# OFA-Sys/ONE-PEACE

Hardware: NVIDIA H100
Metric: encoder_samples_per_sec (higher is better)
Workload: dtype bf16

## Files before the change

one_peace_b200/csrc/gemm_wgmma.cu:

```cuda
#include "common.cuh"
#include "gemm.h"

#include <mutex>

namespace opb {

constexpr int kBlockM = 128;
constexpr int kBlockN = 256;
constexpr int kBlockK = 64;
constexpr int kStages = 4;
constexpr int kABytes = kBlockM * kBlockK * 2;
constexpr int kBBytes = kBlockN * kBlockK * 2;
constexpr int kStageBytes = kABytes + kBBytes;
constexpr int kThreads = 384;
constexpr int kBandM = 8;
constexpr int kResidBatch = 16;

struct EpiOperands {
  float2 row[kBlockM];
  float colsum[kBlockN], bias[kBlockN], gamma[kBlockN], colscale[kBlockN];
};
constexpr int kStagerThreads = 96;
constexpr int kSmemBytes = kStages * kStageBytes + 1024 + 2 * sizeof(EpiOperands) + 1024;

struct GemmGeom {
  int M, N, K;
  int kb_inner;
  int num_k_blocks;
  int groups;
  int a_group_c0;
  int b_group_rows;
  int a_mn;
  int b_mn;
  int kb_per_piece;
  int m_pad;
  float* split_ws;
};

OPB_DEVICE void fence_acc(float (&d)[128]) {
#pragma unroll
  for (int i = 0; i < 128; ++i) asm volatile("" : "+f"(d[i])::"memory");
}

template <int TA, int TB>
OPB_DEVICE void wgmma_m64n256k16(float (&d)[128], uint64_t desc_a, uint64_t desc_b, uint32_t scale_d) {
  asm volatile(
      "{\n\t"
      ".reg .pred p;\n\t"
      "setp.ne.b32 p, %130, 0;\n\t"
      "wgmma.mma_async.sync.aligned.m64n256k16.f32.bf16.bf16 "
      "{"
      "%0, %1, %2, %3, %4, %5, %6, %7, %8, %9, %10, %11, %12, %13, %14, %15, "
      "%16, %17, %18, %19, %20, %21, %22, %23, %24, %25, %26, %27, %28, %29, %30, %31, "
      "%32, %33, %34, %35, %36, %37, %38, %39, %40, %41, %42, %43, %44, %45, %46, %47, "
      "%48, %49, %50, %51, %52, %53, %54, %55, %56, %57, %58, %59, %60, %61, %62, %63, "
      "%64, %65, %66, %67, %68, %69, %70, %71, %72, %73, %74, %75, %76, %77, %78, %79, "
      "%80, %81, %82, %83, %84, %85, %86, %87, %88, %89, %90, %91, %92, %93, %94, %95, "
      "%96, %97, %98, %99, %100, %101, %102, %103, %104, %105, %106, %107, %108, %109, %110, %111, "
      "%112, %113, %114, %115, %116, %117, %118, %119, %120, %121, %122, %123, %124, %125, %126, %127"
      "}, %128, %129, p, 1, 1, %131, %132;\n\t"
      "}\n"
      : "+f"(d[0]), "+f"(d[1]), "+f"(d[2]), "+f"(d[3]), "+f"(d[4]), "+f"(d[5]), "+f"(d[6]), "+f"(d[7]),
        "+f"(d[8]), "+f"(d[9]), "+f"(d[10]), "+f"(d[11]), "+f"(d[12]), "+f"(d[13]), "+f"(d[14]), "+f"(d[15]),
        "+f"(d[16]), "+f"(d[17]), "+f"(d[18]), "+f"(d[19]), "+f"(d[20]), "+f"(d[21]), "+f"(d[22]), "+f"(d[23]),
        "+f"(d[24]), "+f"(d[25]), "+f"(d[26]), "+f"(d[27]), "+f"(d[28]), "+f"(d[29]), "+f"(d[30]), "+f"(d[31]),
        "+f"(d[32]), "+f"(d[33]), "+f"(d[34]), "+f"(d[35]), "+f"(d[36]), "+f"(d[37]), "+f"(d[38]), "+f"(d[39]),
        "+f"(d[40]), "+f"(d[41]), "+f"(d[42]), "+f"(d[43]), "+f"(d[44]), "+f"(d[45]), "+f"(d[46]), "+f"(d[47]),
        "+f"(d[48]), "+f"(d[49]), "+f"(d[50]), "+f"(d[51]), "+f"(d[52]), "+f"(d[53]), "+f"(d[54]), "+f"(d[55]),
        "+f"(d[56]), "+f"(d[57]), "+f"(d[58]), "+f"(d[59]), "+f"(d[60]), "+f"(d[61]), "+f"(d[62]), "+f"(d[63]),
        "+f"(d[64]), "+f"(d[65]), "+f"(d[66]), "+f"(d[67]), "+f"(d[68]), "+f"(d[69]), "+f"(d[70]), "+f"(d[71]),
        "+f"(d[72]), "+f"(d[73]), "+f"(d[74]), "+f"(d[75]), "+f"(d[76]), "+f"(d[77]), "+f"(d[78]), "+f"(d[79]),
        "+f"(d[80]), "+f"(d[81]), "+f"(d[82]), "+f"(d[83]), "+f"(d[84]), "+f"(d[85]), "+f"(d[86]), "+f"(d[87]),
        "+f"(d[88]), "+f"(d[89]), "+f"(d[90]), "+f"(d[91]), "+f"(d[92]), "+f"(d[93]), "+f"(d[94]), "+f"(d[95]),
        "+f"(d[96]), "+f"(d[97]), "+f"(d[98]), "+f"(d[99]), "+f"(d[100]), "+f"(d[101]), "+f"(d[102]), "+f"(d[103]),
        "+f"(d[104]), "+f"(d[105]), "+f"(d[106]), "+f"(d[107]), "+f"(d[108]), "+f"(d[109]), "+f"(d[110]), "+f"(d[111]),
        "+f"(d[112]), "+f"(d[113]), "+f"(d[114]), "+f"(d[115]), "+f"(d[116]), "+f"(d[117]), "+f"(d[118]), "+f"(d[119]),
        "+f"(d[120]), "+f"(d[121]), "+f"(d[122]), "+f"(d[123]), "+f"(d[124]), "+f"(d[125]), "+f"(d[126]), "+f"(d[127])
      : "l"(desc_a), "l"(desc_b), "r"(scale_d), "n"(TA), "n"(TB));
}

template <bool kFusedVar = false>
OPB_DEVICE void load_ln_stats(const GemmEpilogue& ep, int row, int M, float& mu, float& rs) {
  mu = 0.f; rs = 1.f;
  const int rc = row < M ? row : M - 1;
  if (ep.ln_partial != nullptr) {
    float s1 = 0.f, s2 = 0.f;
#pragma unroll 8
    for (int p = 0; p < ep.ln_parts; ++p) {
      const float2 v = *reinterpret_cast<const float2*>(ep.ln_partial + (static_cast<long>(p) * M + rc) * 2);
// ... 20 lines not shown
                         uint32_t it0) {
  constexpr uint32_t step_a = TA ? 2048 : 32, step_b = TB ? 2048 : 32;
  const bool signal = (threadIdx.x & 31) == 0;
  for (int kb = 0; kb < num_k_blocks; ++kb) {
    const uint32_t it = it0 + kb;
    const uint32_t s = it % kStages;
    mbar_wait_quiet(&full[s], (it / kStages) & 1);
    const uint32_t sa = smem_u32(smem + s * kStageBytes) + cw * 8192;
    const uint32_t sb = smem_u32(smem + s * kStageBytes + kABytes);
    fence_acc(d);
    wgmma_fence();
#pragma unroll
    for (int k = 0; k < kBlockK / 16; ++k)
      wgmma_m64n256k16<TA, TB>(d, wgmma_desc_sw128(sa + k * step_a, 8192), wgmma_desc_sw128(sb + k * step_b, 8192),
                               (kb > 0 || k > 0) ? 1u : 0u);
    wgmma_commit();
    fence_acc(d);
    if (kb > 0) {
      wgmma_wait<1>();
      fence_acc(d);
      __syncwarp();
      if (signal) mbar_arrive(&empty[(it - 1) % kStages]);
    }
  }
  wgmma_wait<0>();
  fence_acc(d);
  __syncwarp();
  if (signal) mbar_arrive(&empty[(it0 + num_k_blocks - 1) % kStages]);
}

constexpr bool epi_staged(int epi) { return epi != EPI_LSE_PARTIAL && epi != EPI_SOFTMAX_GRAD; }

template <int EPI>
OPB_DEVICE void stage_epi_operands(EpiOperands* st, const GemmEpilogue& ep, const GemmGeom& geo, int m_blk, int n_blk, int grp,
                                   int t) {
  if (ep.ln_partial != nullptr || ep.ln_mu != nullptr) {
    for (int r = t; r < kBlockM; r += kStagerThreads) {
      float mu, rs;
      load_ln_stats<EPI == EPI_GEGLU_BF16 || EPI == EPI_RESID_F32>(ep, m_blk * kBlockM + r, geo.M, mu, rs);
      st->row[r] = make_float2(mu, rs);
    }
  }
  for (int c = t; c < kBlockN; c += kStagerThreads) {
    const int tc = n_blk * kBlockN + c;
    const bool ok = tc < geo.N;
    const int col = grp * geo.N + tc;
    st->colsum[c] = ok && ep.ln_colsum != nullptr ? ep.ln_colsum[col] : 0.f;
    st->bias[c] = ok && ep.bias != nullptr ? ep.bias[col] : 0.f;
    st->gamma[c] = ok && ep.gamma != nullptr ? ep.gamma[col] : 0.f;
    st->colscale[c] = ok && ep.colscale != nullptr ? ep.colscale[col] : 0.f;
  }
}

template <int EPI>
OPB_DEVICE void epilogue(const float (&d)[128], const GemmEpilogue& ep, const GemmGeom& geo, const EpiOperands* st, int m_blk,
                         int n_blk, int grp, int cw) {
  const int M = geo.M, N = geo.N;
  const int t = threadIdx.x & 127;
  const int lane = t & 31;
  const int quad = lane & 3;
  const int rloc = cw * 64 + (t >> 5) * 16 + (lane >> 2);
  const int rbase = m_blk * kBlockM + rloc;
  const int col0 = n_blk * kBlockN;
  const int gcol0 = grp * N;
#pragma unroll
  for (int h = 0; h < 2; ++h) {
    const int row = rbase + 8 * h;
    bool row_ok = row < M;
    if (ep.out_group > 0 && ep.out_group_valid > 0 && (row % ep.out_group) >= ep.out_group_valid) row_ok = false;
    long out_row = row;
    if (ep.out_group > 0) out_row = static_cast<long>(row / ep.out_group) * ep.out_group_stride + (row % ep.out_group) + ep.out_row_offset;
    long res_row = out_row;
    if (ep.resid_period > 0) res_row = (row % ep.resid_period) + ep.resid_row_offset;

    if constexpr (EPI == EPI_LSE_PARTIAL) {
      const float scale = *ep.scale_ptr;
      const int tgt = row + ep.target_offset;
      const int nv = ep.n_valid > 0 ? ep.n_valid : N;
      float m = -INFINITY;
#pragma unroll
      for (int j = 0; j < 32; ++j) {
        const int col = col0 + 8 * j + 2 * quad;
        if (col < nv) m = fmaxf(m, scale * d[4 * j + 2 * h]);
        if (col + 1 < nv) m = fmaxf(m, scale * d[4 * j + 2 * h + 1]);
      }
      float ssum = 0.f, zsum = 0.f, best = -INFINITY, ztgt = 0.f;
      int best_idx = 0, has_tgt = 0;
#pragma unroll
      for (int j = 0; j < 32; ++j) {
#pragma unroll
        for (int e = 0; e < 2; ++e) {
          const int col = col0 + 8 * j + 2 * quad + e;
          if (col < nv) {
            const float z = scale * d[4 * j + 2 * h + e];
            ssum += __expf(z - m);
            zsum += z;
            if (z > best) { best = z; best_idx = col; }
            if (col == tgt) { ztgt = z; has_tgt = 1; }
          }
        }
      }
#pragma unroll
      for (int o = 1; o <= 2; o <<= 1) {
        const float m2 = __shfl_xor_sync(0xffffffffu, m, o), s2 = __shfl_xor_sync(0xffffffffu, ssum, o);
        const float zs2 = __shfl_xor_sync(0xffffffffu, zsum, o), b2 = __shfl_xor_sync(0xffffffffu, best, o);
        const int i2 = __shfl_xor_sync(0xffffffffu, best_idx, o), h2 = __shfl_xor_sync(0xffffffffu, has_tgt, o);
        const float zt2 = __shfl_xor_sync(0xffffffffu, ztgt, o);
        const float mn = fmaxf(m, m2);
        ssum = (m > -INFINITY ? ssum * __expf(m - mn) : 0.f) + (m2 > -INFINITY ? s2 * __expf(m2 - mn) : 0.f);
        m = mn;
        zsum += zs2;
        if (b2 > best || (b2 == best && i2 < best_idx)) { best = b2; best_idx = i2; }
        if (h2) { ztgt = zt2; has_tgt = 1; }
      }
      if (row_ok && quad == 0) {
        float* w = ep.ws + (static_cast<long>(n_blk) * M + row) * 8;
        *reinterpret_cast<float4*>(w) = make_float4(m, ssum, zsum, best);
        *reinterpret_cast<float4*>(w + 4) = make_float4(__int_as_float(best_idx), ztgt, has_tgt ? 1.f : 0.f, 0.f);
      }
    } else if constexpr (EPI == EPI_SOFTMAX_GRAD) {
      const float scale = *ep.scale_ptr;
      const float gscale = scale * ep.coef;
      const int tgt = row + ep.target_offset;
      const float lse = row_ok ? ep.row_lse[row] : 0.f;
      const float hit = 1.f - ep.eps - ep.eps_i;
      const int nv = ep.n_valid > 0 ? ep.n_valid : N;
      float gz = 0.f;
#pragma unroll
      for (int j = 0; j < 32; ++j) {
        const int col = col0 + 8 * j + 2 * quad;
        if (!row_ok || col >= N) continue;
        float gq[2];
#pragma unroll
        for (int e = 0; e < 2; ++e) {
          const float z = scale * d[4 * j + 2 * h + e];
          float g = __expf(z - lse) - ep.eps_i;
          if (col + e == tgt) g -= hit;
          if (col + e >= nv) g = 0.f;
          gz += g * z;
          gq[e] = g * gscale;
        }
        *reinterpret_cast<uint32_t*>(reinterpret_cast<__nv_bfloat16*>(ep.out) + out_row * ep.ldo + col) = pack_bf16x2(gq[0], gq[1]);
      }
      gz = quad_sum(gz);
      if (row_ok && quad == 0) ep.ws[static_cast<long>(n_blk) * M + row] = gz;
    } else {
      const float2 mr = (ep.ln_partial != nullptr || ep.ln_mu != nullptr) ? st->row[rloc + 8 * h] : make_float2(0.f, 1.f);
      const float mu = mr.x, rs = mr.y;
      const bool has_ln = ep.ln_colsum != nullptr;
      float st_sum = 0.f, st_sq = 0.f;
      if constexpr (EPI == EPI_GEGLU_BF16) {
        __nv_bfloat16* out = reinterpret_cast<__nv_bfloat16*>(ep.out) + out_row * ep.ldo + n_blk * (kBlockN / 2);
#pragma unroll
        for (int j = 0; j < 16; ++j) {
          const int tc = 8 * j + 2 * quad;
          float g0 = d[4 * j + 2 * h], g1 = d[4 * j + 2 * h + 1];
          float l0 = d[4 * (j + 16) + 2 * h], l1 = d[4 * (j + 16) + 2 * h + 1];
          if (has_ln) {
            const float2 cg = ldf2(st->colsum + tc), cl = ldf2(st->colsum + tc + kBlockN / 2);
            g0 = rs * (g0 - mu * cg.x); g1 = rs * (g1 - mu * cg.y);
            l0 = rs * (l0 - mu * cl.x); l1 = rs * (l1 - mu * cl.y);
          }
          if (ep.bias != nullptr) {
            const float2 bg = ldf2(st->bias + tc), bl = ldf2(st->bias + tc + kBlockN / 2);
            g0 += bg.x; g1 += bg.y; l0 += bl.x; l1 += bl.y;
          }
          const float u0 = gelu_erf(g0) * l0, u1 = gelu_erf(g1) * l1;
          st_sum += u0 + u1;
          st_sq += u0 * u0 + u1 * u1;
          if (row_ok) *reinterpret_cast<uint32_t*>(out + tc) = pack_bf16x2(u0, u1);
        }
        st_sum = quad_sum(st_sum);
        st_sq = quad_sum(st_sq);
        if (row_ok && quad == 0 && ep.stats_out != nullptr) {
          *reinterpret_cast<float2*>(ep.stats_out + (static_cast<long>(n_blk * 2) * M + row) * 2) = make_float2(st_sum, st_sq);
          *reinterpret_cast<float2*>(ep.stats_out + (static_cast<long>(n_blk * 2 + 1) * M + row) * 2) = make_float2(0.f, 0.f);
        }
      } else {
#pragma unroll
        for (int jb = 0; jb < 32; jb += kResidBatch) {
          float2 res[kResidBatch];
          if constexpr (EPI == EPI_RESID_F32) {
            if (ep.resid != nullptr && row_ok) {
              const float* rp = ep.resid + res_row * ep.ldr + gcol0;
#pragma unroll
              for (int jj = 0; jj < kResidBatch; ++jj) {
                const int tc = col0 + 8 * (jb + jj) + 2 * quad;
                if (tc < N) res[jj] = ldf2(rp + tc);
              }
            }
          }
#pragma unroll
          for (int jj = 0; jj < kResidBatch; ++jj) {
            const int j = jb + jj;
            const int lc = 8 * j + 2 * quad;
            const int tc = col0 + lc;
            if (tc >= N) continue;
            const int col = gcol0 + tc;
            float x0 = d[4 * j + 2 * h], x1 = d[4 * j + 2 * h + 1];
            if (has_ln) {
              const float2 c = ldf2(st->colsum + lc);
              x0 = rs * (x0 - mu * c.x); x1 = rs * (x1 - mu * c.y);
            }
            if (ep.bias != nullptr) {
              const float2 b = ldf2(st->bias + lc);
              x0 += b.x; x1 += b.y;
            }
            if constexpr (EPI == EPI_STORE_BF16 || EPI == EPI_GELU_BF16) {
              if (ep.colscale != nullptr) {
                const float2 s = ldf2(st->colscale + lc);
                x0 *= s.x; x1 *= s.y;
              }
              if constexpr (EPI == EPI_GELU_BF16) { x0 = gelu_erf(x0); x1 = gelu_erf(x1); }
              if (row_ok) *reinterpret_cast<uint32_t*>(reinterpret_cast<__nv_bfloat16*>(ep.out) + out_row * ep.ldo + col) = pack_bf16x2(x0, x1);
            } else {
              if constexpr (EPI == EPI_RESID_F32) {
                if (ep.gamma != nullptr) {
                  const float2 g = ldf2(st->gamma + lc);
                  x0 *= g.x; x1 *= g.y;
                }
                if (ep.resid != nullptr && row_ok) {
                  x0 += res[jj].x; x1 += res[jj].y;
                }
                st_sum += x0 + x1;
                st_sq += x0 * x0 + x1 * x1;
                if (row_ok && ep.out_bf16 != nullptr)
                  *reinterpret_cast<uint32_t*>(reinterpret_cast<__nv_bfloat16*>(ep.out_bf16) + out_row * ep.ldo_bf16 + col) = pack_bf16x2(x0, x1);
              }
              if (row_ok) *reinterpret_cast<float2*>(reinterpret_cast<float*>(ep.out) + out_row * ep.ldo + col) = make_float2(x0, x1);
            }
          }
        }
        if constexpr (EPI == EPI_RESID_F32) {
          st_sum = quad_sum(st_sum);
          st_sq = quad_sum(st_sq);
          if (row_ok && quad == 0 && ep.stats_out != nullptr)
            *reinterpret_cast<float2*>(ep.stats_out + (static_cast<long>(n_blk) * M + row) * 2) = make_float2(st_sum, st_sq);
        }
      }
    }
  }
}

struct TileCoord {
  int piece, grp, m_blk, n_blk;
};
OPB_DEVICE TileCoord tile_coord(int unit, int num_m_tiles, int num_n_tiles, int groups) {
  const int per_group = num_m_tiles * num_n_tiles;
  TileCoord c;
  c.piece = unit / (per_group * groups);
  const int tile = unit - c.piece * per_group * groups;
  c.grp = tile / per_group;
  const int tin = tile - c.grp * per_group;
  const int band = tin / (kBandM * num_n_tiles);
  const int m0 = band * kBandM;
  const int band_rows = min(kBandM, num_m_tiles - m0);
  const int r = tin - m0 * num_n_tiles;
  c.m_blk = m0 + r % band_rows;
  c.n_blk = r / band_rows;
  return c;
}

template <int EPI>
__global__ void __launch_bounds__(kThreads, 1)
gemm_bf16_kernel(const __grid_constant__ CUtensorMap tm_a, const __grid_constant__ CUtensorMap tm_b, const GemmEpilogue ep,
                 const GemmGeom geo) {
  extern __shared__ __align__(1024) uint8_t smem_raw[];
  uint8_t* smem = smem_raw;
  if ((smem_u32(smem) & 1023u) != 0) __trap();
  uint64_t* full = reinterpret_cast<uint64_t*>(smem + kStages * kStageBytes);
  uint64_t* empty = full + kStages;
  uint64_t* epi_full = empty + kStages;
  uint64_t* epi_empty = epi_full + 2;
  EpiOperands* epi_ops = reinterpret_cast<EpiOperands*>(smem + kStages * kStageBytes + 1024);

  const int wg = threadIdx.x >> 7;
  const int num_m_tiles = (geo.M + kBlockM - 1) / kBlockM;
  const int num_n_tiles = (geo.N + kBlockN - 1) / kBlockN;
  const int pieces = geo.kb_per_piece > 0 ? (geo.num_k_blocks + geo.kb_per_piece - 1) / geo.kb_per_piece : 1;
  const int units = num_m_tiles * num_n_tiles * geo.groups * pieces;
  const bool staged = epi_staged(EPI) && geo.kb_per_piece == 0;

  if (threadIdx.x == 0) {
    tma_prefetch_desc(&tm_a);
    tma_prefetch_desc(&tm_b);
    for (int i = 0; i < kStages; ++i) {
      mbar_init(&full[i], 1);
      mbar_init(&empty[i], 8);
    }
    for (int i = 0; i < 2; ++i) {
      mbar_init(&epi_full[i], kStagerThreads);
      mbar_init(&epi_empty[i], 8);
    }
    fence_barrier_init();
  }
  __syncthreads();

  if (wg == 0) {
    asm volatile("setmaxnreg.dec.sync.aligned.u32 40;");
    if (threadIdx.x == 0) {
      uint32_t it = 0;
      for (int unit = blockIdx.x; unit < units; unit += gridDim.x) {
        const TileCoord tc = tile_coord(unit, num_m_tiles, num_n_tiles, geo.groups);
        const int kb0 = geo.kb_per_piece > 0 ? tc.piece * geo.kb_per_piece : 0;
        const int kb1 = geo.kb_per_piece > 0 ? min(geo.num_k_blocks, kb0 + geo.kb_per_piece) : geo.num_k_blocks;
        const int a_row = tc.m_blk * kBlockM;
        const int b_row = tc.grp * geo.b_group_rows + tc.n_blk * kBlockN;
        const int a_c0 = tc.grp * geo.a_group_c0;
        int kin = kb0 % geo.kb_inner, tap = kb0 / geo.kb_inner;
        for (int kb = kb0; kb < kb1; ++kb, ++it) {
          const uint32_t s = it % kStages;
          mbar_wait_quiet(&empty[s], ((it / kStages) & 1) ^ 1);
          uint8_t* sa = smem + s * kStageBytes;
          uint8_t* sb = sa + kABytes;
          mbar_arrive_expect_tx(&full[s], kStageBytes);
          if (geo.a_mn) {
#pragma unroll
            for (int i = 0; i < kBlockM / 64; ++i) tma_load_2d(&tm_a, &full[s], sa + i * 8192, a_row + 64 * i, kb * kBlockK);
          } else {
            tma_load_3d(&tm_a, &full[s], sa, a_c0 + kin * kBlockK, tap, a_row);
          }
          if (geo.b_mn) {
#pragma unroll
            for (int i = 0; i < kBlockN / 64; ++i) tma_load_2d(&tm_b, &full[s], sb + i * 8192, b_row + 64 * i, kb * kBlockK);
          } else {
            tma_load_2d(&tm_b, &full[s], sb, kb * kBlockK, b_row);
          }
          if (++kin == geo.kb_inner) { kin = 0; ++tap; }
        }
      }
    } else if (threadIdx.x >= 32 && staged) {
      uint32_t j = 0;
      for (int unit = blockIdx.x; unit < units; unit += gridDim.x, ++j) {
        const TileCoord tc = tile_coord(unit, num_m_tiles, num_n_tiles, geo.groups);
        mbar_wait_quiet(&epi_empty[j & 1], ((j >> 1) & 1) ^ 1);
        stage_epi_operands<EPI>(&epi_ops[j & 1], ep, geo, tc.m_blk, tc.n_blk, tc.grp, threadIdx.x - 32);
        mbar_arrive(&epi_full[j & 1]);
      }
    }
  } else {
    asm volatile("setmaxnreg.inc.sync.aligned.u32 232;");
    const int cw = wg - 1;
    float d[128];
#pragma unroll
    for (int i = 0; i < 128; ++i) d[i] = 0.f;
    uint32_t it = 0, j = 0;
    for (int unit = blockIdx.x; unit < units; unit += gridDim.x, ++j) {
      const TileCoord tc = tile_coord(unit, num_m_tiles, num_n_tiles, geo.groups);
      const int kb0 = geo.kb_per_piece > 0 ? tc.piece * geo.kb_per_piece : 0;
      const int kb1 = geo.kb_per_piece > 0 ? min(geo.num_k_blocks, kb0 + geo.kb_per_piece) : geo.num_k_blocks;
      if (geo.a_mn) {
        if (geo.b_mn) mainloop<1, 1>(d, smem, full, empty, kb1 - kb0, cw, it);
        else mainloop<1, 0>(d, smem, full, empty, kb1 - kb0, cw, it);
      } else {
        if (geo.b_mn) mainloop<0, 1>(d, smem, full, empty, kb1 - kb0, cw, it);
        else mainloop<0, 0>(d, smem, full, empty, kb1 - kb0, cw, it);
      }
      it += kb1 - kb0;
      if (geo.kb_per_piece > 0) {
        const int t = threadIdx.x & 127, lane = t & 31;
        const int r0 = tc.m_blk * kBlockM + cw * 64 + (t >> 5) * 16 + (lane >> 2);
        float* w = geo.split_ws + static_cast<long>(tc.piece) * geo.m_pad * geo.N;
#pragma unroll
        for (int h = 0; h < 2; ++h) {
#pragma unroll
          for (int c = 0; c < 32; ++c) {
            const int col = tc.n_blk * kBlockN + 8 * c + 2 * (lane & 3);
            if (col < geo.N)
              *reinterpret_cast<float2*>(w + static_cast<long>(r0 + 8 * h) * geo.N + col) = make_float2(d[4 * c + 2 * h], d[4 * c + 2 * h + 1]);
          }
        }
      } else if (staged) {
        mbar_wait_quiet(&epi_full[j & 1], (j >> 1) & 1);
        epilogue<EPI>(d, ep, geo, &epi_ops[j & 1], tc.m_blk, tc.n_blk, tc.grp, cw);
        __syncwarp();
        if ((threadIdx.x & 31) == 0) mbar_arrive(&epi_empty[j & 1]);
      } else {
        epilogue<EPI>(d, ep, geo, nullptr, tc.m_blk, tc.n_blk, tc.grp, cw);
      }
    }
  }
}

__global__ void __launch_bounds__(256)
gemm_split_epilogue_kernel(const GemmEpilogue ep, const GemmGeom geo, int pieces, int epi) {
  __shared__ float red[2][8];
  const int M = geo.M, N = geo.N;
  const int row = blockIdx.x;
  float mu, rs;
  if (ep.ln_partial != nullptr) {
    float s1 = 0.f, s2 = 0.f;
    for (int p = threadIdx.x; p < ep.ln_parts; p += blockDim.x) {
      const float2 v = *reinterpret_cast<const float2*>(ep.ln_partial + (static_cast<long>(p) * M + row) * 2);
      s1 += v.x; s2 += v.y;
    }
    s1 = warp_sum(s1); s2 = warp_sum(s2);
    if ((threadIdx.x & 31) == 0) { red[0][threadIdx.x >> 5] = s1; red[1][threadIdx.x >> 5] = s2; }
    __syncthreads();
    s1 = s2 = 0.f;
    for (int i = 0; i < 8; ++i) { s1 += red[0][i]; s2 += red[1][i]; }
    mu = s1 / ep.ln_dim;
    rs = rsqrtf(fmaxf(s2 / ep.ln_dim - mu * mu, 0.f) + ep.ln_eps);
  } else {
    load_ln_stats(ep, row, M, mu, rs);
  }
  const int t = blockIdx.y;
  const int col = t * kBlockN + threadIdx.x;
  const long slab = static_cast<long>(geo.m_pad) * N;
  float x = 0.f;
  if (col < N) {
    const float* w = geo.split_ws + static_cast<long>(row) * N + col;
    for (int p = 0; p < pieces; ++p) x += w[p * slab];
    if (ep.ln_colsum) x = rs * (x - mu * ep.ln_colsum[col]);
    if (ep.bias) x += ep.bias[col];
    if (epi == EPI_STORE_BF16) {
      if (ep.colscale) x *= ep.colscale[col];
      reinterpret_cast<__nv_bfloat16*>(ep.out)[static_cast<long>(row) * ep.ldo + col] = __float2bfloat16(x);
    } else {
      if (ep.gamma) x *= ep.gamma[col];
      if (ep.resid) x += ep.resid[static_cast<long>(row) * ep.ldr + col];
      reinterpret_cast<float*>(ep.out)[static_cast<long>(row) * ep.ldo + col] = x;
      if (ep.out_bf16) reinterpret_cast<__nv_bfloat16*>(ep.out_bf16)[static_cast<long>(row) * ep.ldo_bf16 + col] = __float2bfloat16(x);
    }
  }
  if (ep.stats_out != nullptr) {
    const float s1 = warp_sum(x), s2 = warp_sum(x * x);
    __syncthreads();
    if ((threadIdx.x & 31) == 0) { red[0][threadIdx.x >> 5] = s1; red[1][threadIdx.x >> 5] = s2; }
    __syncthreads();
    if (threadIdx.x == 0) {
      float a = 0.f, b = 0.f;
// ... 38 lines not shown

int make_tmap_bf16_3d(CUtensorMap* out, const void* ptr, uint64_t k_inner, uint64_t taps, uint64_t tap_stride,
                      uint64_t rows, uint64_t row_stride, uint32_t box_rows) {
  PFN_encodeTiled enc = get_encode_fn();
  if (enc == nullptr) return OPB_ERR_CUDA;
  if ((reinterpret_cast<uintptr_t>(ptr) & 15) != 0 || (tap_stride * 2) % 16 != 0 || (row_stride * 2) % 16 != 0)
    return OPB_ERR_INVALID;
  cuuint64_t gdim[3] = {k_inner, taps, rows};
  cuuint64_t gstride[2] = {tap_stride * 2, row_stride * 2};
  cuuint32_t box[3] = {static_cast<cuuint32_t>(kBlockK), 1, box_rows};
  cuuint32_t estr[3] = {1, 1, 1};
  CUresult r = enc(out, CU_TENSOR_MAP_DATA_TYPE_BFLOAT16, 3, const_cast<void*>(ptr), gdim, gstride, box, estr,
                   CU_TENSOR_MAP_INTERLEAVE_NONE, CU_TENSOR_MAP_SWIZZLE_128B, CU_TENSOR_MAP_L2_PROMOTION_L2_256B,
                   CU_TENSOR_MAP_FLOAT_OOB_FILL_NONE);
  return r == CUDA_SUCCESS ? OPB_OK : OPB_ERR_CUDA;
}

int make_tmap_bf16_batched(CUtensorMap* out, const void* ptr, uint64_t cols, uint64_t rows, uint64_t ld, uint64_t batches,
                           uint64_t batch_stride, uint32_t box_rows) {
  PFN_encodeTiled enc = get_encode_fn();
  if (enc == nullptr) return OPB_ERR_CUDA;
  if ((reinterpret_cast<uintptr_t>(ptr) & 15) != 0 || (ld * 2) % 16 != 0 || (batch_stride * 2) % 16 != 0)
    return OPB_ERR_INVALID;
  cuuint64_t gdim[3] = {cols, rows, batches};
  cuuint64_t gstride[2] = {ld * 2, batch_stride * 2};
  cuuint32_t box[3] = {static_cast<cuuint32_t>(kBlockK), box_rows, 1};
  cuuint32_t estr[3] = {1, 1, 1};
  CUresult r = enc(out, CU_TENSOR_MAP_DATA_TYPE_BFLOAT16, 3, const_cast<void*>(ptr), gdim, gstride, box, estr,
                   CU_TENSOR_MAP_INTERLEAVE_NONE, CU_TENSOR_MAP_SWIZZLE_128B, CU_TENSOR_MAP_L2_PROMOTION_L2_256B,
                   CU_TENSOR_MAP_FLOAT_OOB_FILL_NONE);
  return r == CUDA_SUCCESS ? OPB_OK : OPB_ERR_CUDA;
}

template <int EPI>
static int launch_gemm(const CUtensorMap& ta, const CUtensorMap& tb, const GemmEpilogue& ep, const GemmGeom& geo,
                       cudaStream_t stream) {
  auto kern = gemm_bf16_kernel<EPI>;
  static int resident = 0;
  if (resident == 0) {
    if (cudaFuncSetAttribute(kern, cudaFuncAttributeMaxDynamicSharedMemorySize, kSmemBytes) != cudaSuccess)
      return OPB_ERR_CUDA;
    int per_sm = 0;
    if (cudaOccupancyMaxActiveBlocksPerMultiprocessor(&per_sm, kern, kThreads, kSmemBytes) != cudaSuccess || per_sm < 1)
      return OPB_ERR_CUDA;
    resident = per_sm * sm_count();
  }
  const int pieces = geo.kb_per_piece > 0 ? (geo.num_k_blocks + geo.kb_per_piece - 1) / geo.kb_per_piece : 1;
  const long units = static_cast<long>((geo.M + kBlockM - 1) / kBlockM) * ((geo.N + kBlockN - 1) / kBlockN) * geo.groups * pieces;
  const unsigned grid = static_cast<unsigned>(units < resident ? units : resident);
  kern<<<grid, kThreads, kSmemBytes, stream>>>(ta, tb, ep, geo);
  return cudaGetLastError() == cudaSuccess ? OPB_OK : OPB_ERR_CUDA;
}

static int dispatch_gemm(int epi, const CUtensorMap& ta, const CUtensorMap& tb, const GemmEpilogue& ep, const GemmGeom& geo,
                         cudaStream_t stream) {
  switch (epi) {
    case EPI_STORE_BF16: return launch_gemm<EPI_STORE_BF16>(ta, tb, ep, geo, stream);
    case EPI_GELU_BF16: return launch_gemm<EPI_GELU_BF16>(ta, tb, ep, geo, stream);
    case EPI_GEGLU_BF16: return launch_gemm<EPI_GEGLU_BF16>(ta, tb, ep, geo, stream);
    case EPI_RESID_F32: return launch_gemm<EPI_RESID_F32>(ta, tb, ep, geo, stream);
    case EPI_STORE_F32: return launch_gemm<EPI_STORE_F32>(ta, tb, ep, geo, stream);
    case EPI_LSE_PARTIAL: return launch_gemm<EPI_LSE_PARTIAL>(ta, tb, ep, geo, stream);
    case EPI_SOFTMAX_GRAD: return launch_gemm<EPI_SOFTMAX_GRAD>(ta, tb, ep, geo, stream);
    default: return OPB_ERR_INVALID;
  }
}

struct ByteSpan {
  const char* begin;
  const char* end;
};
static ByteSpan row_span(const void* p, long lo, long hi, long ld, long cols, int esz) {
  const char* c = static_cast<const char*>(p);
  return {c + lo * ld * esz, c + (hi * ld + cols) * esz};
}
static bool spans_meet(const ByteSpan& a, const ByteSpan& b) { return a.begin < b.end && b.begin < a.end; }

static bool resid_aliasing_ok(const GemmEpilogue& ep, int M, long cols) {
  if (ep.resid == nullptr) return true;
  auto out_row = [&](long m) {
    return ep.out_group > 0 ? (m / ep.out_group) * ep.out_group_stride + m % ep.out_group + ep.out_row_offset : m;
  };
  const long g = ep.out_group > 0 ? ep.out_group : M, last = M - 1, q = last / g;
  const long corners[5] = {0, (g < M ? g : M) - 1, q * g, last, q > 0 ? q * g - 1 : 0};
  long lo = out_row(0), hi = lo;
  for (long m : corners) {
    lo = out_row(m) < lo ? out_row(m) : lo;
    hi = out_row(m) > hi ? out_row(m) : hi;
  }
  long rlo = lo, rhi = hi;
  if (ep.resid_period > 0) {
    rlo = ep.resid_row_offset;
    rhi = rlo + (ep.resid_period < M ? ep.resid_period : M) - 1;
  }
  const ByteSpan res = row_span(ep.resid, rlo, rhi, ep.ldr, cols, 4);
  if (ep.out_bf16 != nullptr && spans_meet(res, row_span(ep.out_bf16, lo, hi, ep.ldo_bf16, cols, 2))) return false;
  if (!spans_meet(res, row_span(ep.out, lo, hi, ep.ldo, cols, 4))) return true;
  return ep.resid == ep.out && ep.ldr == ep.ldo && ep.resid_period == 0;
}

static GemmGeom plain_geom(int M, int N, int K) {
  GemmGeom geo;
  geo.M = M; geo.N = N; geo.K = K;
  geo.num_k_blocks = (K + kBlockK - 1) / kBlockK;
  geo.kb_inner = geo.num_k_blocks;
  geo.groups = 1;
  geo.a_group_c0 = 0;
  geo.b_group_rows = 0;
  geo.a_mn = geo.b_mn = 0;
  geo.kb_per_piece = 0;
  geo.m_pad = 0;
  geo.split_ws = nullptr;
  return geo;
}

int gemm_bf16(const void* A, int lda, const void* B, int ldb, int M, int N, int K, int epi, const GemmEpilogue& ep,
              int cta_group, cudaStream_t stream) {
  if (M <= 0 || N <= 0 || K <= 0) return OPB_ERR_INVALID;
  if (K % 8 != 0 || N % 8 != 0 || lda % 8 != 0 || ldb % 8 != 0) return OPB_ERR_INVALID;
  if (epi == EPI_GEGLU_BF16 && N % kBlockN != 0) return OPB_ERR_INVALID;
  if (cta_group < 0 || cta_group > 2) return OPB_ERR_INVALID;
  if (epi == EPI_RESID_F32 && !resid_aliasing_ok(ep, M, N)) return OPB_ERR_INVALID;
  GemmGeom geo = plain_geom(M, N, K);
  const int m_tiles = (M + kBlockM - 1) / kBlockM, n_tiles = (N + kBlockN - 1) / kBlockN;
  const bool split_ok = (epi == EPI_RESID_F32 || (epi == EPI_STORE_BF16 && ep.stats_out == nullptr)) && ep.workspace != nullptr &&
                        ep.out_group == 0 && ep.resid_period == 0 && M <= 2 * kBlockM && geo.num_k_blocks >= 8;
  int pieces = 1;
  if (split_ok) {
    const long slab_bytes = static_cast<long>(m_tiles) * kBlockM * N * 4;
    pieces = sm_count() / (m_tiles * n_tiles);
    if (pieces > geo.num_k_blocks / 2) pieces = geo.num_k_blocks / 2;
    if (pieces > ep.workspace_bytes / slab_bytes) pieces = static_cast<int>(ep.workspace_bytes / slab_bytes);
    if (pieces >= 2) {
      geo.kb_per_piece = (geo.num_k_blocks + pieces - 1) / pieces;
      pieces = (geo.num_k_blocks + geo.kb_per_piece - 1) / geo.kb_per_piece;
      geo.m_pad = m_tiles * kBlockM;
      geo.split_ws = reinterpret_cast<float*>(ep.workspace);
    }
  }
  CUtensorMap ta, tb;
  int rc = make_tmap_bf16_3d(&ta, A, K, 1, lda, M, lda, kBlockM);
  if (rc != OPB_OK) return rc;
  rc = make_tmap_bf16_2d(&tb, B, N, K, ldb, kBlockN);
  if (rc != OPB_OK) return rc;
  rc = dispatch_gemm(epi, ta, tb, ep, geo, stream);
  if (rc != OPB_OK || geo.kb_per_piece == 0) return rc;
  gemm_split_epilogue_kernel<<<dim3(M, n_tiles), 256, 0, stream>>>(ep, geo, pieces, epi);
  return cudaGetLastError() == cudaSuccess ? OPB_OK : OPB_ERR_CUDA;
}

int gemm_bf16_t(const void* A, int lda, int a_mn, const void* B, int ldb, int b_mn, int M, int N, int K, int epi,
                const GemmEpilogue& ep, int cta_group, cudaStream_t stream) {
  if (M <= 0 || N <= 0 || K <= 0 || lda % 8 != 0 || ldb % 8 != 0 || N % 8 != 0) return OPB_ERR_INVALID;
  if (epi != EPI_STORE_BF16 && epi != EPI_STORE_F32) return OPB_ERR_INVALID;
  if ((!a_mn && K % 8 != 0) || (!b_mn && K % 8 != 0) || (a_mn && M % 8 != 0)) return OPB_ERR_INVALID;
  if (cta_group < 0 || cta_group > 2) return OPB_ERR_INVALID;
  GemmGeom geo = plain_geom(M, N, K);
  geo.a_mn = a_mn ? 1 : 0;
  geo.b_mn = b_mn ? 1 : 0;
  CUtensorMap ta, tb;
  int rc = a_mn ? make_tmap_bf16_2d(&ta, A, K, M, lda, 64) : make_tmap_bf16_3d(&ta, A, K, 1, lda, M, lda, kBlockM);
  if (rc != OPB_OK) return rc;
  rc = b_mn ? make_tmap_bf16_2d(&tb, B, K, N, ldb, 64) : make_tmap_bf16_2d(&tb, B, N, K, ldb, kBlockN);
  if (rc != OPB_OK) return rc;
  return dispatch_gemm(epi, ta, tb, ep, geo, stream);
// ... 25 lines not shown
```

Measured before the change: 760.6.

## Stage GEMM epilogue outputs through swizzled per-warp smem for coalesced 16B stores

```diff
diff --git a/one_peace_b200/csrc/gemm_wgmma.cu b/one_peace_b200/csrc/gemm_wgmma.cu
--- a/one_peace_b200/csrc/gemm_wgmma.cu
+++ b/one_peace_b200/csrc/gemm_wgmma.cu
@@ -1,6 +1,7 @@
 #include "common.cuh"
 #include "gemm.h"
 
+#include <algorithm>
 #include <mutex>
 
 namespace opb {
@@ -14,14 +15,15 @@
 constexpr int kStageBytes = kABytes + kBBytes;
 constexpr int kThreads = 384;
 constexpr int kBandM = 8;
-constexpr int kResidBatch = 16;
 
 struct EpiOperands {
   float2 row[kBlockM];
   float colsum[kBlockN], bias[kBlockN], gamma[kBlockN], colscale[kBlockN];
 };
 constexpr int kStagerThreads = 96;
-constexpr int kSmemBytes = kStages * kStageBytes + 1024 + 2 * sizeof(EpiOperands) + 1024;
+constexpr int kWarpStageBytes = 16 * 128;
+constexpr int kSmemBytes = kStages * kStageBytes + 1024 + 2 * sizeof(EpiOperands) + 8 * kWarpStageBytes + 1024;
+static_assert(kSmemBytes <= 232448, "exceeds the sm_90 opt-in shared memory per block");
 
 struct GemmGeom {
   int M, N, K;
@@ -35,6 +37,7 @@
   int kb_per_piece;
   int m_pad;
   float* split_ws;
+  int vec;
 };
 
 OPB_DEVICE void fence_acc(float (&d)[128]) {
@@ -161,28 +164,79 @@
   }
 }
 
+OPB_DEVICE int stage_off(int r, int byte) {
+  const int swz = ((r & 3) << 1) | ((r >> 2) & 1);
+  return r * 128 + ((((byte >> 4) ^ swz) << 4) | (byte & 15));
+}
+OPB_DEVICE void stage_bf16x2(uint8_t* buf, int r, int jj, int quad, float a, float b) {
+  *reinterpret_cast<uint32_t*>(buf + stage_off(r, jj * 16 + quad * 4)) = pack_bf16x2(a, b);
+}
+OPB_DEVICE void stage_f32x2(uint8_t* buf, int r, int jj, int quad, float a, float b) {
+  *reinterpret_cast<float2*>(buf + stage_off(r, jj * 32 + quad * 8)) = make_float2(a, b);
+}
+
+OPB_DEVICE void st_global_vec(char* p, const uint4& v, int bytes, int vec) {
+  if (vec == 16) {
+    *reinterpret_cast<uint4*>(p) = v;
+    return;
+  }
+  const uint32_t w[4] = {v.x, v.y, v.z, v.w};
+#pragma unroll
+  for (int i = 0; i < 4; ++i) {
+    if (4 * i >= bytes) break;
+    if (vec == 8) {
+      if ((i & 1) == 0) *reinterpret_cast<uint2*>(p + 4 * i) = make_uint2(w[i], w[i + 1]);
+    } else {
+      *reinterpret_cast<uint32_t*>(p + 4 * i) = w[i];
+    }
+  }
+}
+
+OPB_DEVICE void unstage(const uint8_t* buf, int drow, char* out, long ld, int valid, int vec,
+                        char* out_bf16 = nullptr, long ld_bf16 = 0) {
+  const int lane = threadIdx.x & 31;
+  const int b = (lane & 7) * 16;
+  __syncwarp();
+#pragma unroll
+  for (int i = 0; i < 4; ++i) {
+    const int r = 4 * i + (lane >> 3);
+    const uint4 v = *reinterpret_cast<const uint4*>(buf + stage_off(r, b));
+    const int orow = __shfl_sync(0xffffffffu, drow, r);
+    if (orow < 0 || b >= valid) continue;
+    st_global_vec(out + static_cast<long>(orow) * ld + b, v, 16, vec);
+    if (out_bf16 != nullptr) {
+      const uint4 h = make_uint4(pack_bf16x2(__uint_as_float(v.x), __uint_as_float(v.y)),
+                                 pack_bf16x2(__uint_as_float(v.z), __uint_as_float(v.w)), 0u, 0u);
+      st_global_vec(out_bf16 + static_cast<long>(orow) * ld_bf16 + b / 2, h, 8, vec / 2);
+    }
+  }
+  __syncwarp();
+}
+
+OPB_DEVICE int out_row_of(const GemmEpilogue& ep, int row, int M) {
+  if (row >= M) return -1;
+  if (ep.out_group <= 0) return row;
+  if (ep.out_group_valid > 0 && row % ep.out_group >= ep.out_group_valid) return -1;
+  return (row / ep.out_group) * ep.out_group_stride + row % ep.out_group + ep.out_row_offset;
+}
+
 template <int EPI>
-OPB_DEVICE void epilogue(const float (&d)[128], const GemmEpilogue& ep, const GemmGeom& geo, const EpiOperands* st, int m_blk,
-                         int n_blk, int grp, int cw) {
+OPB_DEVICE void epilogue(const float (&d)[128], const GemmEpilogue& ep, const GemmGeom& geo, const EpiOperands* st,
+                         uint8_t* stage, int m_blk, int n_blk, int grp, int cw) {
   const int M = geo.M, N = geo.N;
   const int t = threadIdx.x & 127;
   const int lane = t & 31;
   const int quad = lane & 3;
-  const int rloc = cw * 64 + (t >> 5) * 16 + (lane >> 2);
-  const int rbase = m_blk * kBlockM + rloc;
+  const int r0 = lane >> 2;
+  const int wrow = cw * 64 + (t >> 5) * 16;
+  const int rbase = m_blk * kBlockM + wrow + r0;
   const int col0 = n_blk * kBlockN;
   const int gcol0 = grp * N;
-#pragma unroll
-  for (int h = 0; h < 2; ++h) {
-    const int row = rbase + 8 * h;
-    bool row_ok = row < M;
-    if (ep.out_group > 0 && ep.out_group_valid > 0 && (row % ep.out_group) >= ep.out_group_valid) row_ok = false;
-    long out_row = row;
-    if (ep.out_group > 0) out_row = static_cast<long>(row / ep.out_group) * ep.out_group_stride + (row % ep.out_group) + ep.out_row_offset;
-    long res_row = out_row;
-    if (ep.resid_period > 0) res_row = (row % ep.resid_period) + ep.resid_row_offset;
-
-    if constexpr (EPI == EPI_LSE_PARTIAL) {
+  if constexpr (EPI == EPI_LSE_PARTIAL) {
+#pragma unroll
+    for (int h = 0; h < 2; ++h) {
+      const int row = rbase + 8 * h;
+      const bool row_ok = out_row_of(ep, row, M) >= 0;
       const float scale = *ep.scale_ptr;
       const int tgt = row + ep.target_offset;
       const int nv = ep.n_valid > 0 ? ep.n_valid : N;
@@ -227,128 +281,213 @@
         *reinterpret_cast<float4*>(w) = make_float4(m, ssum, zsum, best);
         *reinterpret_cast<float4*>(w + 4) = make_float4(__int_as_float(best_idx), ztgt, has_tgt ? 1.f : 0.f, 0.f);
       }
-    } else if constexpr (EPI == EPI_SOFTMAX_GRAD) {
+    }
+  } else {
+    const int drow = out_row_of(ep, m_blk * kBlockM + wrow + (lane & 15), M);
+    int frow[2];
+#pragma unroll
+    for (int h = 0; h < 2; ++h) frow[h] = out_row_of(ep, rbase + 8 * h, M);
+    if constexpr (EPI == EPI_SOFTMAX_GRAD) {
       const float scale = *ep.scale_ptr;
       const float gscale = scale * ep.coef;
-      const int tgt = row + ep.target_offset;
-      const float lse = row_ok ? ep.row_lse[row] : 0.f;
       const float hit = 1.f - ep.eps - ep.eps_i;
       const int nv = ep.n_valid > 0 ? ep.n_valid : N;
-      float gz = 0.f;
-#pragma unroll
-      for (int j = 0; j < 32; ++j) {
-        const int col = col0 + 8 * j + 2 * quad;
-        if (!row_ok || col >= N) continue;
-        float gq[2];
-#pragma unroll
-        for (int e = 0; e < 2; ++e) {
-          const float z = scale * d[4 * j + 2 * h + e];
-          float g = __expf(z - lse) - ep.eps_i;
-          if (col + e == tgt) g -= hit;
-          if (col + e >= nv) g = 0.f;
-          gz += g * z;
-          gq[e] = g * gscale;
+      float lse[2], gz[2] = {0.f, 0.f};
+#pragma unroll
+      for (int h = 0; h < 2; ++h) lse[h] = frow[h] >= 0 ? ep.row_lse[rbase + 8 * h] : 0.f;
+      char* out = static_cast<char*>(ep.out) + static_cast<long>(gcol0 + col0) * 2;
+#pragma unroll
+      for (int c = 0; c < 4; ++c) {
+#pragma unroll
+        for (int jj = 0; jj < 8; ++jj) {
+          const int j = 8 * c + jj;
+          const int col = col0 + 8 * j + 2 * quad;
+#pragma unroll
+          for (int h = 0; h < 2; ++h) {
+            if (frow[h] < 0 || col >= N) continue;
+            const int tgt = rbase + 8 * h + ep.target_offset;
+            float gq[2];
+#pragma unroll
+            for (int e = 0; e < 2; ++e) {
+              const float z = scale * d[4 * j + 2 * h + e];
+              float g = __expf(z - lse[h]) - ep.eps_i;
+              if (col + e == tgt) g -= hit;
+              if (col + e >= nv) g = 0.f;
+              gz[h] += g * z;
+              gq[e] = g * gscale;
+            }
+            stage_bf16x2(stage, r0 + 8 * h, jj, quad, gq[0], gq[1]);
+          }
         }
-        *reinterpret_cast<uint32_t*>(reinterpret_cast<__nv_bfloat16*>(ep.out) + out_row * ep.ldo + col) = pack_bf16x2(gq[0], gq[1]);
-      }
-      gz = quad_sum(gz);
-      if (row_ok && quad == 0) ep.ws[static_cast<long>(n_blk) * M + row] = gz;
+        unstage(stage, drow, out + c * 128, ep.ldo * 2, (N - col0 - 64 * c) * 2, geo.vec);
+      }
+#pragma unroll
+      for (int h = 0; h < 2; ++h) {
+        const float s = quad_sum(gz[h]);
+        if (frow[h] >= 0 && quad == 0) ep.ws[static_cast<long>(n_blk) * M + rbase + 8 * h] = s;
+      }
     } else {
-      const float2 mr = (ep.ln_partial != nullptr || ep.ln_mu != nullptr) ? st->row[rloc + 8 * h] : make_float2(0.f, 1.f);
-      const float mu = mr.x, rs = mr.y;
+      const bool has_row = ep.ln_partial != nullptr || ep.ln_mu != nullptr;
+      float mu[2], rs[2];
+#pragma unroll
+      for (int h = 0; h < 2; ++h) {
+        const float2 mr = has_row ? st->row[wrow + r0 + 8 * h] : make_float2(0.f, 1.f);
+        mu[h] = mr.x; rs[h] = mr.y;
+      }
       const bool has_ln = ep.ln_colsum != nullptr;
-      float st_sum = 0.f, st_sq = 0.f;
+      float st_sum[2] = {0.f, 0.f}, st_sq[2] = {0.f, 0.f};
       if constexpr (EPI == EPI_GEGLU_BF16) {
-        __nv_bfloat16* out = reinterpret_cast<__nv_bfloat16*>(ep.out) + out_row * ep.ldo + n_blk * (kBlockN / 2);
-#pragma unroll
-        for (int j = 0; j < 16; ++j) {
-          const int tc = 8 * j + 2 * quad;
-          float g0 = d[4 * j + 2 * h], g1 = d[4 * j + 2 * h + 1];
-          float l0 = d[4 * (j + 16) + 2 * h], l1 = d[4 * (j + 16) + 2 * h + 1];
-          if (has_ln) {
-            const float2 cg = ldf2(st->colsum + tc), cl = ldf2(st->colsum + tc + kBlockN / 2);
-            g0 = rs * (g0 - mu * cg.x); g1 = rs * (g1 - mu * cg.y);
-            l0 = rs * (l0 - mu * cl.x); l1 = rs * (l1 - mu * cl.y);
-          }
-          if (ep.bias != nullptr) {
-            const float2 bg = ldf2(st->bias + tc), bl = ldf2(st->bias + tc + kBlockN / 2);
-            g0 += bg.x; g1 += bg.y; l0 += bl.x; l1 += bl.y;
-          }
-          const float u0 = gelu_erf(g0) * l0, u1 = gelu_erf(g1) * l1;
-          st_sum += u0 + u1;
-          st_sq += u0 * u0 + u1 * u1;
-          if (row_ok) *reinterpret_cast<uint32_t*>(out + tc) = pack_bf16x2(u0, u1);
+        char* out = static_cast<char*>(ep.out) + n_blk * (kBlockN / 2) * 2;
+#pragma unroll
+        for (int c = 0; c < 2; ++c) {
+#pragma unroll
+          for (int jj = 0; jj < 8; ++jj) {
+            const int j = 8 * c + jj;
+            const int tc = 8 * j + 2 * quad;
+#pragma unroll
+            for (int h = 0; h < 2; ++h) {
+              float g0 = d[4 * j + 2 * h], g1 = d[4 * j + 2 * h + 1];
+              float l0 = d[4 * (j + 16) + 2 * h], l1 = d[4 * (j + 16) + 2 * h + 1];
+              if (has_ln) {
+                const float2 cg = ldf2(st->colsum + tc), cl = ldf2(st->colsum + tc + kBlockN / 2);
+                g0 = rs[h] * (g0 - mu[h] * cg.x); g1 = rs[h] * (g1 - mu[h] * cg.y);
+                l0 = rs[h] * (l0 - mu[h] * cl.x); l1 = rs[h] * (l1 - mu[h] * cl.y);
+              }
+              if (ep.bias != nullptr) {
+                const float2 bg = ldf2(st->bias + tc), bl = ldf2(st->bias + tc + kBlockN / 2);
+                g0 += bg.x; g1 += bg.y; l0 += bl.x; l1 += bl.y;
+              }
+              const float u0 = gelu_erf(g0) * l0, u1 = gelu_erf(g1) * l1;
+              st_sum[h] += u0 + u1;
+              st_sq[h] += u0 * u0 + u1 * u1;
+              stage_bf16x2(stage, r0 + 8 * h, jj, quad, u0, u1);
+            }
+          }
+          unstage(stage, drow, out + c * 128, ep.ldo * 2, 128, geo.vec);
         }
-        st_sum = quad_sum(st_sum);
-        st_sq = quad_sum(st_sq);
-        if (row_ok && quad == 0 && ep.stats_out != nullptr) {
-          *reinterpret_cast<float2*>(ep.stats_out + (static_cast<long>(n_blk * 2) * M + row) * 2) = make_float2(st_sum, st_sq);
-          *reinterpret_cast<float2*>(ep.stats_out + (static_cast<long>(n_blk * 2 + 1) * M + row) * 2) = make_float2(0.f, 0.f);
+#pragma unroll
+        for (int h = 0; h < 2; ++h) {
+          const int row = rbase + 8 * h;
+          const float s1 = quad_sum(st_sum[h]), s2 = quad_sum(st_sq[h]);
+          if (frow[h] >= 0 && quad == 0 && ep.stats_out != nullptr) {
+            *reinterpret_cast<float2*>(ep.stats_out + (static_cast<long>(n_blk * 2) * M + row) * 2) = make_float2(s1, s2);
+            *reinterpret_cast<float2*>(ep.stats_out + (static_cast<long>(n_blk * 2 + 1) * M + row) * 2) = make_float2(0.f, 0.f);
+          }
         }
-      } else {
-#pragma unroll
-        for (int jb = 0; jb < 32; jb += kResidBatch) {
-          float2 res[kResidBatch];
-          if constexpr (EPI == EPI_RESID_F32) {
-            if (ep.resid != nullptr && row_ok) {
-              const float* rp = ep.resid + res_row * ep.ldr + gcol0;
-#pragma unroll
-              for (int jj = 0; jj < kResidBatch; ++jj) {
-                const int tc = col0 + 8 * (jb + jj) + 2 * quad;
-                if (tc < N) res[jj] = ldf2(rp + tc);
+      } else if constexpr (EPI == EPI_STORE_BF16 || EPI == EPI_GELU_BF16) {
+        char* out = static_cast<char*>(ep.out) + static_cast<long>(gcol0 + col0) * 2;
+#pragma unroll
+        for (int c = 0; c < 4; ++c) {
+#pragma unroll
+          for (int jj = 0; jj < 8; ++jj) {
+            const int j = 8 * c + jj;
+            const int lc = 8 * j + 2 * quad;
+            if (col0 + lc >= N) continue;
+#pragma unroll
+            for (int h = 0; h < 2; ++h) {
+              float x0 = d[4 * j + 2 * h], x1 = d[4 * j + 2 * h + 1];
+              if (has_ln) {
+                const float2 cs = ldf2(st->colsum + lc);
+                x0 = rs[h] * (x0 - mu[h] * cs.x); x1 = rs[h] * (x1 - mu[h] * cs.y);
               }
-            }
-          }
-#pragma unroll
-          for (int jj = 0; jj < kResidBatch; ++jj) {
-            const int j = jb + jj;
-            const int lc = 8 * j + 2 * quad;
-            const int tc = col0 + lc;
-            if (tc >= N) continue;
-            const int col = gcol0 + tc;
-            float x0 = d[4 * j + 2 * h], x1 = d[4 * j + 2 * h + 1];
-            if (has_ln) {
-              const float2 c = ldf2(st->colsum + lc);
-              x0 = rs * (x0 - mu * c.x); x1 = rs * (x1 - mu * c.y);
-            }
-            if (ep.bias != nullptr) {
-              const float2 b = ldf2(st->bias + lc);
-              x0 += b.x; x1 += b.y;
-            }
-            if constexpr (EPI == EPI_STORE_BF16 || EPI == EPI_GELU_BF16) {
+              if (ep.bias != nullptr) {
+                const float2 b = ldf2(st->bias + lc);
+                x0 += b.x; x1 += b.y;
+              }
               if (ep.colscale != nullptr) {
                 const float2 s = ldf2(st->colscale + lc);
                 x0 *= s.x; x1 *= s.y;
               }
               if constexpr (EPI == EPI_GELU_BF16) { x0 = gelu_erf(x0); x1 = gelu_erf(x1); }
-              if (row_ok) *reinterpret_cast<uint32_t*>(reinterpret_cast<__nv_bfloat16*>(ep.out) + out_row * ep.ldo + col) = pack_bf16x2(x0, x1);
-            } else {
+              stage_bf16x2(stage, r0 + 8 * h, jj, quad, x0, x1);
+            }
+          }
+          unstage(stage, drow, out + c * 128, ep.ldo * 2, (N - col0 - 64 * c) * 2, geo.vec);
+        }
+      } else {
+        char* out = static_cast<char*>(ep.out) + static_cast<long>(gcol0 + col0) * 4;
+        char* out_bf16 = nullptr;
+        if constexpr (EPI == EPI_RESID_F32)
+          if (ep.out_bf16 != nullptr) out_bf16 = static_cast<char*>(ep.out_bf16) + static_cast<long>(gcol0 + col0) * 2;
+        const float* rp[2];
+#pragma unroll
+        for (int h = 0; h < 2; ++h) {
+          const int res_row = ep.resid_period > 0 ? (rbase + 8 * h) % ep.resid_period + ep.resid_row_offset : frow[h];
+          rp[h] = ep.resid != nullptr && frow[h] >= 0 ? ep.resid + static_cast<long>(res_row) * ep.ldr + gcol0 : nullptr;
+        }
+        float2 res[2][2][4];
+#pragma unroll
+        for (int c = 0; c < 8; ++c) {
+          if constexpr (EPI == EPI_RESID_F32) {
+#pragma unroll
+            for (int cl = c; c % 2 == 0 && cl <= c + 1; ++cl) {
+#pragma unroll
+              for (int h = 0; h < 2; ++h) {
+                if (rp[h] == nullptr) continue;
+#pragma unroll
+                for (int jj = 0; jj < 4; ++jj) {
+                  const int tc = col0 + 8 * (4 * cl + jj) + 2 * quad;
+                  if (tc < N) res[cl & 1][h][jj] = ldf2(rp[h] + tc);
+                }
+              }
+            }
+          }
+#pragma unroll
+          for (int jj = 0; jj < 4; ++jj) {
+            const int j = 4 * c + jj;
+            const int lc = 8 * j + 2 * quad;
+            if (col0 + lc >= N) continue;
+#pragma unroll
+            for (int h = 0; h < 2; ++h) {
+              float x0 = d[4 * j + 2 * h], x1 = d[4 * j + 2 * h + 1];
+              if (has_ln) {
+                const float2 cs = ldf2(st->colsum + lc);
+                x0 = rs[h] * (x0 - mu[h] * cs.x); x1 = rs[h] * (x1 - mu[h] * cs.y);
+              }
+              if (ep.bias != nullptr) {
+                const float2 b = ldf2(st->bias + lc);
+                x0 += b.x; x1 += b.y;
+              }
               if constexpr (EPI == EPI_RESID_F32) {
                 if (ep.gamma != nullptr) {
                   const float2 g = ldf2(st->gamma + lc);
                   x0 *= g.x; x1 *= g.y;
                 }
-                if (ep.resid != nullptr && row_ok) {
-                  x0 += res[jj].x; x1 += res[jj].y;
+                if (rp[h] != nullptr) {
+                  x0 += res[c & 1][h][jj].x; x1 += res[c & 1][h][jj].y;
                 }
-                st_sum += x0 + x1;
-                st_sq += x0 * x0 + x1 * x1;
-                if (row_ok && ep.out_bf16 != nullptr)
-                  *reinterpret_cast<uint32_t*>(reinterpret_cast<__nv_bfloat16*>(ep.out_bf16) + out_row * ep.ldo_bf16 + col) = pack_bf16x2(x0, x1);
+                st_sum[h] += x0 + x1;
+                st_sq[h] += x0 * x0 + x1 * x1;
               }
-              if (row_ok) *reinterpret_cast<float2*>(reinterpret_cast<float*>(ep.out) + out_row * ep.ldo + col) = make_float2(x0, x1);
+              stage_f32x2(stage, r0 + 8 * h, jj, quad, x0, x1);
             }
           }
+          unstage(stage, drow, out + c * 128, ep.ldo * 4, (N - col0 - 32 * c) * 4, geo.vec,
+                  out_bf16 != nullptr ? out_bf16 + c * 64 : nullptr, ep.ldo_bf16 * 2);
         }
         if constexpr (EPI == EPI_RESID_F32) {
-          st_sum = quad_sum(st_sum);
-          st_sq = quad_sum(st_sq);
-          if (row_ok && quad == 0 && ep.stats_out != nullptr)
-            *reinterpret_cast<float2*>(ep.stats_out + (static_cast<long>(n_blk) * M + row) * 2) = make_float2(st_sum, st_sq);
+#pragma unroll
+          for (int h = 0; h < 2; ++h) {
+            const float s1 = quad_sum(st_sum[h]), s2 = quad_sum(st_sq[h]);
+            if (frow[h] >= 0 && quad == 0 && ep.stats_out != nullptr)
+              *reinterpret_cast<float2*>(ep.stats_out + (static_cast<long>(n_blk) * M + rbase + 8 * h) * 2) = make_float2(s1, s2);
+          }
         }
       }
     }
   }
+}
+
+OPB_DEVICE void prefetch_resid_l2(const GemmEpilogue& ep, const GemmGeom& geo, int m_blk, int n_blk, int grp, int cw) {
+  const int lane = threadIdx.x & 31;
+  const int row = m_blk * kBlockM + cw * 64 + ((threadIdx.x & 127) >> 5) * 16 + (lane & 15);
+  const int orow = out_row_of(ep, row, geo.M);
+  if (orow < 0) return;
+  const int res_row = ep.resid_period > 0 ? row % ep.resid_period + ep.resid_row_offset : orow;
+  const float* p = ep.resid + static_cast<long>(res_row) * ep.ldr + grp * geo.N + n_blk * kBlockN;
+#pragma unroll
+  for (int i = lane >> 4; i < kBlockN / 32; i += 2)
+    if (n_blk * kBlockN + 32 * i < geo.N) asm volatile("prefetch.global.L2 [%0];" ::"l"(p + 32 * i));
 }
 
 struct TileCoord {
@@ -450,6 +589,7 @@
   } else {
     asm volatile("setmaxnreg.inc.sync.aligned.u32 232;");
     const int cw = wg - 1;
+    uint8_t* stage = reinterpret_cast<uint8_t*>(epi_ops + 2) + ((threadIdx.x - 128) >> 5) * kWarpStageBytes;
     float d[128];
 #pragma unroll
     for (int i = 0; i < 128; ++i) d[i] = 0.f;
@@ -458,6 +598,8 @@
       const TileCoord tc = tile_coord(unit, num_m_tiles, num_n_tiles, geo.groups);
       const int kb0 = geo.kb_per_piece > 0 ? tc.piece * geo.kb_per_piece : 0;
       const int kb1 = geo.kb_per_piece > 0 ? min(geo.num_k_blocks, kb0 + geo.kb_per_piece) : geo.num_k_blocks;
+      if constexpr (EPI == EPI_RESID_F32)
+        if (geo.kb_per_piece == 0 && ep.resid != nullptr) prefetch_resid_l2(ep, geo, tc.m_blk, tc.n_blk, tc.grp, cw);
       if (geo.a_mn) {
         if (geo.b_mn) mainloop<1, 1>(d, smem, full, empty, kb1 - kb0, cw, it);
         else mainloop<1, 0>(d, smem, full, empty, kb1 - kb0, cw, it);
@@ -467,25 +609,28 @@
       }
       it += kb1 - kb0;
       if (geo.kb_per_piece > 0) {
-        const int t = threadIdx.x & 127, lane = t & 31;
-        const int r0 = tc.m_blk * kBlockM + cw * 64 + (t >> 5) * 16 + (lane >> 2);
-        float* w = geo.split_ws + static_cast<long>(tc.piece) * geo.m_pad * geo.N;
-#pragma unroll
-        for (int h = 0; h < 2; ++h) {
-#pragma unroll
-          for (int c = 0; c < 32; ++c) {
-            const int col = tc.n_blk * kBlockN + 8 * c + 2 * (lane & 3);
-            if (col < geo.N)
-              *reinterpret_cast<float2*>(w + static_cast<long>(r0 + 8 * h) * geo.N + col) = make_float2(d[4 * c + 2 * h], d[4 * c + 2 * h + 1]);
-          }
+        const int lane = threadIdx.x & 31;
+        const int wrow = tc.m_blk * kBlockM + cw * 64 + ((threadIdx.x & 127) >> 5) * 16;
+        const int drow = wrow + (lane & 15);
+        const int col0 = tc.n_blk * kBlockN;
+        char* w = reinterpret_cast<char*>(geo.split_ws + static_cast<long>(tc.piece) * geo.m_pad * geo.N + col0);
+#pragma unroll
+        for (int c = 0; c < 8; ++c) {
+#pragma unroll
+          for (int jj = 0; jj < 4; ++jj) {
+#pragma unroll
+            for (int h = 0; h < 2; ++h)
+              stage_f32x2(stage, (lane >> 2) + 8 * h, jj, lane & 3, d[4 * (4 * c + jj) + 2 * h], d[4 * (4 * c + jj) + 2 * h + 1]);
+          }
+          unstage(stage, drow, w + c * 128, static_cast<long>(geo.N) * 4, (geo.N - col0 - 32 * c) * 4, geo.vec);
         }
       } else if (staged) {
         mbar_wait_quiet(&epi_full[j & 1], (j >> 1) & 1);
-        epilogue<EPI>(d, ep, geo, &epi_ops[j & 1], tc.m_blk, tc.n_blk, tc.grp, cw);
+        epilogue<EPI>(d, ep, geo, &epi_ops[j & 1], stage, tc.m_blk, tc.n_blk, tc.grp, cw);
         __syncwarp();
         if ((threadIdx.x & 31) == 0) mbar_arrive(&epi_empty[j & 1]);
       } else {
-        epilogue<EPI>(d, ep, geo, nullptr, tc.m_blk, tc.n_blk, tc.grp, cw);
+        epilogue<EPI>(d, ep, geo, nullptr, stage, tc.m_blk, tc.n_blk, tc.grp, cw);
       }
     }
   }
@@ -630,8 +775,26 @@
   return cudaGetLastError() == cudaSuccess ? OPB_OK : OPB_ERR_CUDA;
 }
 
-static int dispatch_gemm(int epi, const CUtensorMap& ta, const CUtensorMap& tb, const GemmEpilogue& ep, const GemmGeom& geo,
+static int store_vec_bytes(int epi, const GemmEpilogue& ep, const GemmGeom& geo) {
+  auto widest = [](const void* p, long pitch_bytes) {
+    const uintptr_t a = reinterpret_cast<uintptr_t>(p) | static_cast<uintptr_t>(pitch_bytes);
+    return (a & 15) == 0 ? 16 : (a & 7) == 0 ? 8 : (a & 3) == 0 ? 4 : 0;
+  };
+  if (geo.kb_per_piece > 0) {
+    const int v = widest(geo.split_ws, static_cast<long>(geo.N) * 4);
+    return v >= 8 ? v : 0;
+  }
+  if (epi == EPI_LSE_PARTIAL) return 16;
+  const bool f32 = epi == EPI_RESID_F32 || epi == EPI_STORE_F32;
+  int v = widest(ep.out, ep.ldo * (f32 ? 4 : 2));
+  if (epi == EPI_RESID_F32 && ep.out_bf16 != nullptr) v = std::min(v, 2 * widest(ep.out_bf16, ep.ldo_bf16 * 2));
+  return v >= (f32 ? 8 : 4) ? v : 0;
+}
+
+static int dispatch_gemm(int epi, const CUtensorMap& ta, const CUtensorMap& tb, const GemmEpilogue& ep, GemmGeom geo,
                          cudaStream_t stream) {
+  geo.vec = store_vec_bytes(epi, ep, geo);
+  if (geo.vec == 0) return OPB_ERR_INVALID;
   switch (epi) {
     case EPI_STORE_BF16: return launch_gemm<EPI_STORE_BF16>(ta, tb, ep, geo, stream);
     case EPI_GELU_BF16: return launch_gemm<EPI_GELU_BF16>(ta, tb, ep, geo, stream);
@@ -689,6 +852,7 @@
   geo.kb_per_piece = 0;
   geo.m_pad = 0;
   geo.split_ws = nullptr;
+  geo.vec = 16;
   return geo;
 }
 
```

Measured after the change: 794.9, median of 6. 4.5% higher.
